# piotrmwojcik/GI-GS

Measured on AMD Instinct MI355X. Metric: train-step renders/sec (fwd+bwd, G-buffer+indirect) at 800x800; PSNR vs the CPU oracle, higher is better.
Workload: dtype f32; 1 GPU; C2 (configs[1] TensoIR lego stand-in): 300k surface Gaussians, 800x800, SH deg 2, GI step=16 start=8 delta=0.0625; P=300000, N=640000, M=9, hip_graphs=on, fused_glue=on, gi_march=proj, rasterizer=whole step = 2 hand-captured hipGraphs (fwd, bwd), asynchronous binning

## Files before the change

gi-gs_amd/csrc/api.hip:

```cpp
#include <cstdarg>
#include <cstdio>
#include <cstdlib>
#include <cstring>
#include <map>
#include <algorithm>
#include <new>
#include <mutex>
#include <vector>

#include "../../include/gigs_hip.h"
#include "gigs_common.h"

namespace {

thread_local char g_err[512] = "";

int fail(int code, const char* fmt, ...) {
  va_list ap;
  va_start(ap, fmt);
  vsnprintf(g_err, sizeof(g_err), fmt, ap);
  va_end(ap);
  return code;
}

// ... 67 lines not shown
  const char* b = getenv("GIGS_BINNING");
  o.binning_legacy = (b && strcmp(b, "legacy") == 0) ? 1 : 0;
  o.bucket_max_mean = env_int("GIGS_BUCKET_MAX_MEAN", gigs::kBucketMaxMeanList);
  const char* ll = getenv("GIGS_LONG_LISTS");
  o.long_lists = (ll && ll[0]) ? (ll[0] == '1' ? 1 : 0) : -1;
  o.bucket_target = std::max(256, env_int("GIGS_BUCKET_TARGET", 1536));
  o.bin_bands = std::max(0, env_int("GIGS_BIN_BANDS", 0));
  o.blend_cull = env_int("GIGS_BLEND_CULL", 1) != 0;
  o.pre_bwd_sh_skip = env_int("GIGS_PRE_BWD_SH_SKIP", 1) != 0;
  o.gi_march = 4;
  if (const char* e = getenv("GIGS_GI_MARCH")) {
    if (strcmp(e, "exact") == 0) o.gi_march = 0;
  }
  o.gi_cert = env_int("GIGS_GI_CERT", 1) != 0;
  o.gi_interleave = env_int("GIGS_GI_INTERLEAVE", 1) != 0;
  o.gi_tile_log2w = env_int("GIGS_GI_TILE_LOG2W", 3);
  if (o.gi_tile_log2w < 0 || o.gi_tile_log2w > 6) o.gi_tile_log2w = 3;
  o.gi_zero_rays = env_int("GIGS_GI_ZERO_RAYS", 0) != 0;
  o.spec_max8 = env_int("GIGS_SPEC_MAX8", 128);
  o.spec_max16 = env_int("GIGS_SPEC_MAX16", 1500);
  o.shade_lds_floats = env_int("GIGS_SHADE_LDS_FLOATS", 30 * 1024);
  o.shade_bwd_blocks = std::max(0, env_int("GIGS_SHADE_BWD_BLOCKS", 0));
  o.shade_bwd_rows = env_int("GIGS_SHADE_BWD_ROWS", 0) != 0;
  return o;
}
const gigs::Ctx& ctx_of(const gigs_ctx* c) { return c ? *reinterpret_cast<const gigs::Ctx*>(c) : gigs::default_ctx(); }

struct ProfRec { int stage; hipEvent_t a, b; };
std::mutex g_prof_mu;
bool g_prof_on = false;
std::vector<ProfRec> g_prof_recs;
std::vector<hipEvent_t> g_prof_pool;

hipEvent_t prof_event() {
  if (!g_prof_pool.empty()) {
    hipEvent_t e = g_prof_pool.back();
    g_prof_pool.pop_back();
    return e;
  }
  hipEvent_t e;
  hipEventCreate(&e);
  return e;
}

struct StageScope {
  hipStream_t s;
// ... 81 lines not shown
  char* p = base;
  gigs::ImageState s = gigs::ImageState::fromChunk(p, N, T);
  const void* ptrs[] = {s.final_T, s.n_contrib, s.ranges, s.tile_order};
  if (which < 0 || which >= 4) return -1;
  return (long long)((const char*)ptrs[which] - base);
}

gigs_ctx* gigs_ctx_create(void) {
  gigs::Ctx* c = new (std::nothrow) gigs::Ctx(gigs::default_ctx());
  if (!c) fail(GIGS_ERR_ALLOC, "gigs_ctx_create: out of host memory");
  return reinterpret_cast<gigs_ctx*>(c);
}
void gigs_ctx_destroy(gigs_ctx* ctx) { delete reinterpret_cast<gigs::Ctx*>(ctx); }

int gigs_ctx_get_options(const gigs_ctx* ctx, gigs_options* out) {
  if (!out || out->struct_bytes < (int)sizeof(gigs_options)) return fail(GIGS_ERR_INVALID, "gigs_ctx_get_options: set struct_bytes = sizeof(gigs_options)");
  const gigs::Options& o = ctx_of(ctx).opt;
  out->struct_bytes = (int)sizeof(gigs_options);
  out->binning_legacy = o.binning_legacy; out->bucket_max_mean = o.bucket_max_mean; out->long_lists = o.long_lists;
  out->bucket_target = o.bucket_target; out->bin_bands = o.bin_bands; out->blend_cull = o.blend_cull; out->pre_bwd_sh_skip = o.pre_bwd_sh_skip;
  out->gi_march = o.gi_march; out->gi_cert = o.gi_cert; out->gi_interleave = o.gi_interleave;
  out->gi_tile_log2w = o.gi_tile_log2w; out->gi_zero_rays = o.gi_zero_rays; out->spec_max8 = o.spec_max8;
  out->spec_max16 = o.spec_max16; out->shade_lds_floats = o.shade_lds_floats; out->shade_bwd_blocks = o.shade_bwd_blocks;
  out->shade_bwd_rows = o.shade_bwd_rows;
  return 0;
}
int gigs_ctx_set_options(gigs_ctx* ctx, const gigs_options* in) {
  if (!ctx) return fail(GIGS_ERR_INVALID, "gigs_ctx_set_options: the default context is immutable, create one");
  if (!in || in->struct_bytes < (int)sizeof(gigs_options)) return fail(GIGS_ERR_INVALID, "gigs_ctx_set_options: set struct_bytes = sizeof(gigs_options)");
  if (in->gi_march != 0 && in->gi_march != 4) return fail(GIGS_ERR_INVALID, "gi_march must be 0 (exact) or 4 (proj)");
  if (in->gi_tile_log2w < 0 || in->gi_tile_log2w > 6) return fail(GIGS_ERR_INVALID, "gi_tile_log2w must be 0..6");
  if (in->long_lists < -1 || in->long_lists > 1) return fail(GIGS_ERR_INVALID, "long_lists must be -1, 0 or 1");
  if (in->bucket_target < 256 || in->bucket_max_mean < 0 || in->bin_bands < 0 || in->bin_bands > 64)
    return fail(GIGS_ERR_INVALID, "bucket_target >= 256, bucket_max_mean >= 0, 0 <= bin_bands <= 64");
  if (in->spec_max8 < 0 || in->spec_max16 < in->spec_max8) return fail(GIGS_ERR_INVALID, "0 <= spec_max8 <= spec_max16");
  if (in->shade_lds_floats < 0 || in->shade_bwd_blocks < 0) return fail(GIGS_ERR_INVALID, "shade_lds_floats, shade_bwd_blocks >= 0");
  gigs::Options& o = reinterpret_cast<gigs::Ctx*>(ctx)->opt;
  o.binning_legacy = in->binning_legacy != 0; o.bucket_max_mean = in->bucket_max_mean; o.long_lists = in->long_lists;
  o.bucket_target = in->bucket_target; o.bin_bands = in->bin_bands; o.blend_cull = in->blend_cull != 0; o.pre_bwd_sh_skip = in->pre_bwd_sh_skip != 0;
  o.gi_march = in->gi_march; o.gi_cert = in->gi_cert != 0; o.gi_interleave = in->gi_interleave != 0;
  o.gi_tile_log2w = in->gi_tile_log2w; o.gi_zero_rays = in->gi_zero_rays != 0; o.spec_max8 = in->spec_max8;
  o.spec_max16 = in->spec_max16; o.shade_lds_floats = in->shade_lds_floats; o.shade_bwd_blocks = in->shade_bwd_blocks;
  o.shade_bwd_rows = in->shade_bwd_rows != 0;
  return 0;
}
int gigs_ctx_set_reuse_binning(gigs_ctx* ctx, int on) {
  if (!ctx) return fail(GIGS_ERR_INVALID, "gigs_ctx_set_reuse_binning: the default context is immutable, create one");
  reinterpret_cast<gigs::Ctx*>(ctx)->reuse_binning = on != 0;
  return 0;
}
int gigs_ctx_set_split_sh(gigs_ctx* ctx, const float* sh_rest) {
  if (!ctx) return fail(GIGS_ERR_INVALID, "gigs_ctx_set_split_sh: the default context is immutable, create one");
  reinterpret_cast<gigs::Ctx*>(ctx)->sh_rest = sh_rest;
  return 0;
}
int gigs_ctx_set_materials_only(gigs_ctx* ctx, void* violations) {
  if (!ctx) return fail(GIGS_ERR_INVALID, "gigs_ctx_set_materials_only: the default context is immutable, create one");
  reinterpret_cast<gigs::Ctx*>(ctx)->materials_only = reinterpret_cast<unsigned*>(violations);
  return 0;
}
int gigs_ctx_set_blend_begin_event(gigs_ctx* ctx, void* hip_event) {
  if (!ctx) return fail(GIGS_ERR_INVALID, "gigs_ctx_set_blend_begin_event: the default context is immutable, create one");
  reinterpret_cast<gigs::Ctx*>(ctx)->blend_begin_event = hip_event;
  return 0;
}

// ... 499 lines not shown
```

gi-gs_amd/csrc/gigs_common.h:

```cpp
#pragma once
#include <hip/hip_runtime.h>
#include <stdint.h>

#define GIGS_BLOCK_X 16
#define GIGS_BLOCK_Y 16
#define GIGS_TILE (GIGS_BLOCK_X * GIGS_BLOCK_Y)
#define GIGS_BREC_F4 5
#define GIGS_GREC 20

namespace gigs {

struct v3 { float x, y, z; };
struct v4 { float x, y, z, w; };

__device__ __forceinline__ v3 operator+(v3 a, v3 b) { return {a.x + b.x, a.y + b.y, a.z + b.z}; }
__device__ __forceinline__ v3 operator-(v3 a, v3 b) { return {a.x - b.x, a.y - b.y, a.z - b.z}; }
__device__ __forceinline__ v3 operator*(v3 a, float s) { return {a.x * s, a.y * s, a.z * s}; }
__device__ __forceinline__ float dot3(v3 a, v3 b) { return a.x * b.x + a.y * b.y + a.z * b.z; }
__device__ __forceinline__ v3 cross3(v3 a, v3 b) {
  return {a.y * b.z - a.z * b.y, a.z * b.x - a.x * b.z, a.x * b.y - a.y * b.x};
}
__device__ __forceinline__ v3 normalize3(v3 v) {
  float inv = 1.0f / sqrtf(dot3(v, v));
  return v * inv;
// ... 162 lines not shown
inline size_t required_bytes(A... a) {
  char* p = nullptr;
  S::fromChunk(p, a...);
  return reinterpret_cast<size_t>(p) + kAlign;
}

struct Options {
  int binning_legacy;
  int bucket_max_mean;
  int long_lists;
  int bucket_target;
  int bin_bands;
  int blend_cull;
  int pre_bwd_sh_skip;
  int gi_march;
  int gi_cert;
  int gi_interleave;
  int gi_tile_log2w;
  int gi_zero_rays;
  int spec_max8, spec_max16;
  int shade_lds_floats;
  int shade_bwd_blocks;
  int shade_bwd_rows;
};
struct Ctx {
  Options opt;
  unsigned async_capacity;
  unsigned* async_counters;
  void* blend_begin_event;
  int reuse_binning;
  unsigned* materials_only;
  const float* sh_rest;
};
const Options& default_options();
const Ctx& default_ctx();

struct FwdArgs {
  int P, D, M, W, H;
  unsigned gx, gy;
  float focal_x, focal_y, tan_fovx, tan_fovy, scale_modifier;
  const float *means3D, *shs, *colors_precomp, *opacities, *normal, *albedo, *roughness,
      *metallic, *scales, *rotations, *cov3D_precomp, *viewmatrix, *projmatrix, *cam_pos,
      *background;
  int argmax_depth, inference;
  const float* shs_rest;
};
// ... 72 lines not shown
```

gi-gs_amd/csrc/pbr.hip:

```cpp
#include <cmath>
#include <cstdlib>
#include <cstring>
#include <map>
#include <mutex>
#include <vector>

#include "gigs_common.h"
#include "pixel_ops.h"

namespace gigs {

__device__ __forceinline__ v3 safe_normalize(v3 v) {
  const float l = sqrtf(v.x * v.x + v.y * v.y + v.z * v.z);
  return l > 0.0f ? v3{v.x / l, v.y / l, v.z / l} : v3{0, 0, 0};
}
__device__ __forceinline__ v3 cube_dir_raw(float fx, float fy, int side) {
  switch (side) {
    case 0: return {1, -fy, -fx};
    case 1: return {-1, -fy, fx};
    case 2: return {fx, 1, fy};
    case 3: return {fx, -1, -fy};
    case 4: return {fx, -fy, 1};
    default: return {-fx, -fy, -1};
  }
// ... 449 lines not shown
static int spec_lanes_for(const Options& o, int avg_window) {
  return (avg_window > 0 && avg_window <= o.spec_max8) ? 8 : (avg_window > 0 && avg_window <= o.spec_max16) ? 16 : 64;
}

template <bool kBackward, bool kNorm>
static void launch_specular_apply(const Options& o, int res, int avg_window, const float* src, const float* bounds,
                                  const uint32_t* offsets, const float* W, float* dst, float* wsum_out, hipStream_t s) {
  const int total = 6 * res * res;
  const int max8 = o.spec_max8, max16 = o.spec_max16;
  if (avg_window > 0 && avg_window <= max8) {
    const int waves = (total + 7) / 8;
    hipLaunchKernelGGL((specular_apply_kernel<kBackward, kNorm, 8>), dim3((waves + 3) / 4), dim3(256), 0, s, res, src,
                       bounds, offsets, W, dst, wsum_out);
  } else if (avg_window > 0 && avg_window <= max16) {
    const int waves = (total + 3) / 4;
    hipLaunchKernelGGL((specular_apply_kernel<kBackward, kNorm, 16>), dim3((waves + 3) / 4), dim3(256), 0, s, res, src,
                       bounds, offsets, W, dst, wsum_out);
  } else {
    hipLaunchKernelGGL((specular_apply_kernel<kBackward, kNorm, 64>), dim3((total + 3) / 4), dim3(256), 0, s, res, src,
                       bounds, offsets, W, dst, wsum_out);
  }
}

__device__ __forceinline__ int cube_face_uv(float x, float y, float z, float& u, float& v) {
  const float ax = fabsf(x), ay = fabsf(y), az = fabsf(z);
  int idx;
  float c;
  if (az > fmaxf(ax, ay)) { idx = 4; c = z; }
  else if (ay > ax) { idx = 2; c = y; y = z; }
  else { idx = 0; c = x; x = z; }
  if (c < 0.f) idx += 1;
  const float m = (1.0f / fabsf(c)) * 0.5f;
  const float m0 = (idx == 0 || idx == 5) ? -m : m;
  const float m1 = (idx != 2) ? -m : m;
  u = x * m0 + 0.5f;
  v = y * m1 + 0.5f;
  if (!isfinite(u) || !isfinite(v)) return -1;
  u = fminf(fmaxf(u, 0.f), 1.f);
  v = fminf(fmaxf(v, 0.f), 1.f);
  return idx;
}

struct Taps { int idx[4]; float w[4]; };

__device__ __forceinline__ bool cube_taps(int res, float dx, float dy, float dz, Taps& t) {
  float u, v;
// ... 802 lines not shown
  if (n_levels <= 0 || n_levels > 8 || !levels) return gigs_internal_fail(GIGS_ERR_INVALID, "specular_cubemap_multi_w: bad level count");
  gigs::SpecLevels L;
  L.n = n_levels;
  int blocks = 0;
  for (int i = 0; i < n_levels; i++) {
    const gigs_spec_level& a = levels[i];
    if (a.res <= 0 || !a.src || !a.bounds || !a.offsets || !a.weights || !a.dst || (!backward && !a.wsum))
      return gigs_internal_fail(GIGS_ERR_INVALID, "specular_cubemap_multi_w: bad level");
    gigs::SpecLevel& v = L.lv[i];
    v.N = a.res; v.lanes = gigs::spec_lanes_for(o, a.avg_window); v.block_begin = blocks;
    v.src = a.src; v.bounds = a.bounds; v.offsets = a.offsets; v.W = a.weights; v.dst = a.dst; v.wsum_out = a.wsum;
    const int total = 6 * a.res * a.res;
    const int waves = v.lanes == 64 ? total : (total + (64 / v.lanes) - 1) / (64 / v.lanes);
    blocks += (waves + 3) / 4;
  }
  void* tok; gigs_internal_stage_begin(backward ? 17 : 16, stream, &tok);
  if (backward) hipLaunchKernelGGL(gigs::specular_apply_multi_kernel<true>, dim3(blocks), dim3(256), 0, (hipStream_t)stream, L);
  else hipLaunchKernelGGL(gigs::specular_apply_multi_kernel<false>, dim3(blocks), dim3(256), 0, (hipStream_t)stream, L);
  gigs_internal_stage_end(tok);
  PBR_CHECK_LAUNCH();
  return 0;
}

int gigs_cubemap_mip_fwd(int res_out, int channels, const float* in, float* out, void* stream) {
  if (res_out <= 0 || channels <= 0 || !in || !out) return gigs_internal_fail(GIGS_ERR_INVALID, "cubemap_mip_fwd: bad argument");
  void* tok; gigs_internal_stage_begin(16, stream, &tok);
  hipLaunchKernelGGL(gigs::cubemap_mip_fwd_kernel, dim3((6 * res_out * res_out * channels + 255) / 256), dim3(256), 0, (hipStream_t)stream, res_out, channels, in, out);
  gigs_internal_stage_end(tok);
  PBR_CHECK_LAUNCH();
  return 0;
}

int gigs_cubemap_mip_bwd(int res_out, const float* dout, float* din, void* stream) {
  if (res_out <= 0 || !dout || !din) return gigs_internal_fail(GIGS_ERR_INVALID, "cubemap_mip_bwd: bad argument");
  const int res = 2 * res_out;
  void* tok; gigs_internal_stage_begin(17, stream, &tok);
  hipLaunchKernelGGL(gigs::cubemap_mip_bwd_kernel, dim3((6 * res * res + 255) / 256), dim3(256), 0, (hipStream_t)stream, res_out, dout, din, (const float*)nullptr,
                     (const float*)nullptr);
  gigs_internal_stage_end(tok);
  PBR_CHECK_LAUNCH();
  return 0;
}

int gigs_cubemap_mip_bwd_add(int res_out, const float* dout, const float* add, float* din, void* stream) {
  if (res_out <= 0 || !dout || !add || !din) return gigs_internal_fail(GIGS_ERR_INVALID, "cubemap_mip_bwd_add: bad argument");
  const int res = 2 * res_out;
// ... 268 lines not shown
```

gi-gs_amd/gigs_lib.py:

```python
from __future__ import annotations

import ctypes as C
import functools
import os
import threading

_HERE = os.path.dirname(os.path.abspath(__file__))
LIB_PATH = os.environ.get("GIGS_LIB", os.path.join(_HERE, "libgigs_hip.so"))

ALLOC_FN = C.CFUNCTYPE(C.c_void_p, C.c_size_t, C.c_void_p)

_f = C.c_void_p
_i = C.c_int
_fl = C.c_float

SIGNATURES = {
    "gigs_last_error": (C.c_char_p, []),
    "gigs_build_arch": (C.c_char_p, []),
    "gigs_required_geom": (C.c_size_t, [_i]),
    "gigs_required_image": (C.c_size_t, [_i, _i]),
    "gigs_required_binning": (C.c_size_t, [_i]),
    "gigs_forward": (_i, [C.c_void_p, ALLOC_FN, C.c_void_p, ALLOC_FN, C.c_void_p, ALLOC_FN, C.c_void_p,
                          _i, _i, _i, _f, _i, _i,
                          _f, _f, _f, _f, _f, _f, _f, _f,
# ... 26 lines not shown
                      C.c_void_p]),
    "gigs_gi_scratch_bytes": (C.c_size_t, [_i, _i]),
    "gigs_ssao_ex": (_i, [C.c_void_p, _i, _i, _fl, _fl, _fl, _fl, _fl, _fl, _i, _i, _f, _f, _f, _f, C.c_void_p]),
    "gigs_ssr_ex": (_i, [C.c_void_p, _i, _i, _fl, _fl, _fl, _fl, _fl, _fl, _i, _i, _f, _f, _f, _f, _f, _f, _f, _f, _f, _f,
                         C.c_void_p]),
    "gigs_ssr_hits": (_i, [C.c_void_p, _i, _i, _fl, _fl, _fl, _fl, _fl, _fl, _i, _i, _f, _f, _f, _f, _f, _f, _f, _f, _f,
                           _i, _f, _f, _f, C.c_uint, _f, C.c_void_p]),
    "gigs_ssr_multi": (_i, [C.c_void_p, _i, _i, _i, _fl, _fl, _fl, _fl, _fl, _fl, _i, _i, _f, _f, _f, _f, _f, _f, _f, _f, _f,
                            _f, C.c_void_p]),
    "gigs_ssr_apply": (_i, [_i, _i, _fl, _f, _f, _f, _f, _f, _f, _f, _f, _f, _f, C.c_void_p]),
    "gigs_median3x3": (_i, [_i, _i, _i, _f, _f, C.c_void_p]),
    "gigs_median3x3_backward": (_i, [_i, _i, _i, _f, _f, _f, C.c_void_p]),
    "gigs_bilateral3x3": (_i, [_i, _i, _i, _fl, _fl, _fl, _f, _f, C.c_void_p]),
    "gigs_diffuse_cubemap_fwd": (_i, [_i, _f, _f, C.c_void_p]),
    "gigs_diffuse_cubemap_bwd": (_i, [_i, _f, _f, C.c_void_p]),
    "gigs_specular_bounds": (_i, [_i, _fl, _f, C.c_void_p]),
    "gigs_specular_cubemap_fwd": (_i, [_i, _f, _f, _fl, _fl, _f, C.c_void_p]),
    "gigs_specular_cubemap_bwd": (_i, [_i, _f, _f, _fl, _fl, _f, C.c_void_p]),
    "gigs_specular_weights": (_i, [_i, _f, _f, _fl, _fl, _i, _f, C.c_void_p]),
    "gigs_specular_weights_divide": (_i, [_i, _f, _f, _f, _f, _f, C.c_void_p]),
    "gigs_specular_cubemap_fwd_w": (_i, [C.c_void_p, _i, _f, _f, _f, _f, _i, _f, _f, C.c_void_p]),
    "gigs_specular_cubemap_bwd_w": (_i, [C.c_void_p, _i, _f, _f, _f, _i, _f, _i, _f, C.c_void_p]),
    "gigs_specular_cubemap_multi_w": (_i, [C.c_void_p, _i, C.c_void_p, _i, C.c_void_p]),
    "gigs_cubemap_mip_fwd": (_i, [_i, _i, _f, _f, C.c_void_p]),
    "gigs_cubemap_mip_bwd_add": (_i, [_i, _f, _f, _f, C.c_void_p]),
    "gigs_cubemap_mip_bwd_add2": (_i, [_i, _f, _f, _f, _f, C.c_void_p]),
    "gigs_cubemap_mip_bwd": (_i, [_i, _f, _f, C.c_void_p]),
    "gigs_shade_fwd": (_i, [_i, _i, _f, _f, _f, _f, _f, _f, _f, _f, _f, _i, _i, C.POINTER(C.c_void_p),
                            C.POINTER(C.c_int), _f, _i, _i, _i, _i, _f, _f, _f, _f, C.c_void_p]),
    "gigs_shade_bwd": (_i, [_i, _i, _f, _f, _f, _f, _f, _f, _f, _f, _i, _i, C.POINTER(C.c_void_p),
                            C.POINTER(C.c_int), _f, _i, _i, _i, _i, _f, _f, _f, _f, _f, _f, _f, _f,
                            C.POINTER(C.c_void_p), C.c_void_p]),
    "gigs_shade_fwd_ex": (_i, [C.c_void_p, _i, _i, _f, _f, _f, _f, _f, _f, _f, _f, _f, _i, _i, C.POINTER(C.c_void_p),
                               C.POINTER(C.c_int), _f, _i, _i, _i, _i, _f, _f, _f, _f, C.c_void_p, C.c_void_p]),
    "gigs_shade_fwd_multi": (_i, [C.c_void_p, _i, _i, _i, _f, _f, _f, _f, _f, _f, _f, C.POINTER(C.c_void_p), _i, _i,
                                  C.POINTER(C.c_void_p), C.POINTER(C.c_int), _f, _i, _i, _i, _i, _f, _f, C.c_void_p]),
    "gigs_shade_bwd_ex": (_i, [C.c_void_p, _i, _i, _f, _f, _f, _f, _f, _f, _f, _f, _i, _i, C.POINTER(C.c_void_p),
                               C.POINTER(C.c_int), _f, _i, _i, _i, _i, _f, _f, _f, _f, _f, _f, _f, _f,
                               C.POINTER(C.c_void_p), C.c_void_p, C.c_void_p]),
    "gigs_gbuffer_post": (_i, [_i, _i, _f, _f, _f, _f, _f, _f, _f, C.c_void_p]),
    "gigs_gbuffer_post_pad": (_i, [_i, _i, _f, _f, _f, _f, _f, _f, _f, _f, _f, _f, _f, _f, C.c_void_p]),
    "gigs_gbuffer_post_bwd": (_i, [_i, _i, _f, _f, _f, _f, _f, C.c_void_p]),
    "gigs_normalize_mask": (_i, [_i, _i, _f, _f, _f, C.c_void_p]),
    "gigs_nonzero_mask": (_i, [_i, _i, _f, _f, C.c_void_p]),
    "gigs_stage2_loss_fwd": (_i, [_i, _i, _f, _f, _f, _f, _f, _f, _f, _f, _f, C.c_void_p]),
    "gigs_stage2_loss_bwd": (_i, [_i, _i, _f, _f, _f, _f, _f, _f, _f, _f, _f, _f, C.c_void_p]),
# ... 44 lines not shown
    "gigs_stream_delay": (_i, [C.c_uint, C.c_void_p]),
    "gigs_ctx_set_async_binning": (_i, [C.c_void_p, _i, C.c_void_p]),
    "gigs_ctx_create": (C.c_void_p, []),
    "gigs_ctx_destroy": (None, [C.c_void_p]),
    "gigs_ctx_get_options": (_i, [C.c_void_p, C.c_void_p]),
    "gigs_ctx_set_options": (_i, [C.c_void_p, C.c_void_p]),
    "gigs_profile_begin": (None, []),
    "gigs_profile_end": (_i, [C.POINTER(C.c_float), C.POINTER(C.c_int), _i]),
    "gigs_profile_stage_name": (C.c_char_p, [_i]),
}

class ShadeExt(C.Structure):
    _fields_ = [("planar", C.c_int), ("rough_scale", C.c_float), ("rough_bias", C.c_float),
                ("out_F0", C.c_void_p), ("out_linear", C.c_void_p), ("out_roughness", C.c_void_p),
                ("g_albedo_mul_a", C.c_void_p), ("g_albedo_mul_b", C.c_void_p),
                ("g_roughness_add", C.c_void_p), ("g_metallic_add", C.c_void_p),
                ("g_scale", C.c_void_p), ("lamb_mask", C.c_void_p), ("lamb_acc4", C.c_void_p)]


class Options(C.Structure):
    _fields_ = [(n, C.c_int) for n in (
        "struct_bytes", "binning_legacy", "bucket_max_mean", "long_lists", "bucket_target", "bin_bands", "blend_cull",
        "pre_bwd_sh_skip", "gi_march", "gi_cert", "gi_interleave", "gi_tile_log2w", "gi_zero_rays", "spec_max8",
        "spec_max16", "shade_lds_floats", "shade_bwd_blocks", "shade_bwd_rows")]


OPTION_NAMES = tuple(n for n, _ in Options._fields_ if n != "struct_bytes")
GI_MARCHES = {0: "exact", 4: "proj"}
_GI_MARCH_VALUES = {name: value for value, name in GI_MARCHES.items()}


class SpecLevel(C.Structure):
    _fields_ = [("res", C.c_int), ("avg_window", C.c_int), ("src", C.c_void_p), ("bounds", C.c_void_p),
                ("offsets", C.c_void_p), ("weights", C.c_void_p), ("dst", C.c_void_p), ("wsum", C.c_void_p)]


class AdamGroup(C.Structure):
    _fields_ = [("param", C.c_void_p), ("grad", C.c_void_p), ("exp_avg", C.c_void_p), ("exp_avg_sq", C.c_void_p),
                ("n", C.c_longlong), ("lr", C.c_double), ("step", C.c_int)]


class ActivationRaw(C.Structure):
    _fields_ = [(n, C.c_void_p) for n in ("f_dc", "f_rest", "opacity", "normal", "albedo", "roughness", "metallic",
                                          "scaling", "rotation")]


class ActivationOut(C.Structure):
    _fields_ = [(n, C.c_void_p) for n in ("shs", "opacities", "normal", "albedo", "roughness", "metallic", "scales",
                                          "rotations")]


class GatherTensor(C.Structure):
    _fields_ = [("src", C.c_void_p), ("dst", C.c_void_p), ("row_floats", C.c_int), ("zero_new", C.c_int)]


class PackDesc(C.Structure):
    _fields_ = [("src", C.c_void_p), ("dst", C.c_void_p), ("lohi", C.c_void_p), ("channels", C.c_int), ("height", C.c_int),
                ("width", C.c_int), ("dst_x", C.c_int), ("dst_stride", C.c_int), ("bias", C.c_float)]


class FilterDesc(C.Structure):
    _fields_ = [("sheet", C.c_void_p), ("out", C.c_void_p), ("height", C.c_int), ("width", C.c_int), ("stride", C.c_int),
                ("reserved", C.c_int)]


MAX_IMAGES = 4096
MINMAX_SCRATCH_FLOATS = 512

_lib = None


class GigsError(RuntimeError):
    pass


def lib():
    global _lib
    if _lib is None:
        if not os.path.exists(LIB_PATH):
            raise ImportError(
                f"{LIB_PATH} not found: build it with `python gi-gs_amd/build.py` "
                "(hipcc, --offload-arch=gfx950). There is no CPU fallback.")
        l = C.CDLL(LIB_PATH)
        for name, (res, args) in SIGNATURES.items():
            fn = getattr(l, name)
            fn.restype = res
            fn.argtypes = args
        _lib = l
# ... 179 lines not shown
```

gi-gs_amd/pbr/renderutils/ops.py:

```python
from __future__ import annotations

import os

import numpy as np
import torch

import gigs_lib

_lib = gigs_lib.lib()


def _stream() -> int:
    return torch.cuda.current_stream().cuda_stream


def _gpu(t: torch.Tensor, name: str) -> torch.Tensor:
    if not t.is_cuda:
        raise RuntimeError(f"{name} must be a CUDA/HIP tensor: pbr.renderutils (gigs-hip) has no CPU path")
    return t.contiguous().float()


class _diffuse_cubemap_func(torch.autograd.Function):
    @staticmethod
    def forward(ctx, cubemap):
# ... 145 lines not shown
        dev = cs[0].device
        outs, wsums, arr = [], [], (gigs_lib.SpecLevel * len(cs))()
        for i, (c, (bounds, tables)) in enumerate(zip(cs, meta)):
            res = c.shape[1]
            out = torch.empty((6, res, res, 3), dtype=torch.float32, device=dev)
            wsum = torch.empty((6, res, res, 1), dtype=torch.float32, device=dev)
            outs.append(out)
            wsums.append(wsum)
            arr[i] = gigs_lib.SpecLevel(res, _avg_window(tables, res), c.data_ptr(), bounds.data_ptr(), tables[0].data_ptr(),
                                        tables[1].data_ptr(), out.data_ptr(), wsum.data_ptr())
        with torch.cuda.device(dev):
            gigs_lib.check(_lib.gigs_specular_cubemap_multi_w(gigs_lib.ctx_ptr(), len(cs), C.cast(arr, C.c_void_p), 0, _stream()),
                           "specular_cubemap_multi_w")
        ctx.meta = meta
        ctx.lib_ctx = gigs_lib.current()
        ctx.shapes = [c.shape[1] for c in cs]
        return tuple(outs)

    @staticmethod
    @gigs_lib.with_forward_context
    def backward(ctx, *douts):
        import ctypes as C
        dev = next(d for d in douts if d is not None).device
        gs, arr, keep = [], (gigs_lib.SpecLevel * len(douts))(), []
        for i, (d, res, (bounds, tables)) in enumerate(zip(douts, ctx.shapes, ctx.meta)):
            d = torch.zeros((6, res, res, 3), dtype=torch.float32, device=dev) if d is None else _gpu(d, "dout")
            keep.append(d)
            g = torch.empty((6, res, res, 3), dtype=torch.float32, device=dev)
            gs.append(g)
            arr[i] = gigs_lib.SpecLevel(res, _avg_window(tables, res), d.data_ptr(), bounds.data_ptr(), tables[0].data_ptr(),
                                        tables[3].data_ptr(), g.data_ptr(), None)
        with torch.cuda.device(dev):
            if bwd_head_start_ns > 0:
                gigs_lib.check(_lib.gigs_stream_delay(int(bwd_head_start_ns), _stream()), "stream_delay")
            gigs_lib.check(_lib.gigs_specular_cubemap_multi_w(gigs_lib.ctx_ptr(), len(douts), C.cast(arr, C.c_void_p), 1, _stream()),
                           "specular_cubemap_multi_w")
        return (None, *gs)


def specular_cubemap_levels(mips, roughnesses, cutoff=0.99):
    if os.environ.get("GIGS_SPEC_MULTI", "1") != "1" or torch.is_anomaly_enabled() or not mips[0].is_cuda:
        return None
    meta = []
    for m, r in zip(mips, roughnesses):
        _, bounds = _ndf_bounds(m.shape[1], r, cutoff, m.device)
        tables = _weight_tables(m.shape[1], r, cutoff, m.device)
        if tables is None or len(tables) < 4 or tables[3] is None:
            return None
        meta.append((bounds, tables))
    return list(_specular_levels.apply(meta, *mips))


_TABLE_MAX_BYTES = float(os.environ.get("GIGS_SPEC_TABLE_MAX_GB", "8")) * 1e9
_weightTables = {}


def _weight_tables(res, roughness, cutoff, device):
    key = (res, roughness, cutoff, str(device))
    if key not in _weightTables:
        cos_cut, bounds = _ndf_bounds(res, roughness, cutoff, device)
        b = bounds.view(-1, 6, 4)
        w = torch.where(b[..., 0] <= b[..., 1], b[..., 1] - b[..., 0] + 1, torch.zeros_like(b[..., 0]))
        h = torch.where(b[..., 2] <= b[..., 3], b[..., 3] - b[..., 2] + 1, torch.zeros_like(b[..., 0]))
        cnt = (w * h).to(torch.int64).reshape(-1)
        total = int(cnt.sum().item())
        used = sum(t[1].numel() * (12 if t[3] is not None else 8) for t in _weightTables.values() if t is not None)
        if total == 0 or total >= 2 ** 31 or used + total * 8 > _TABLE_MAX_BYTES:
            _weightTables[key] = None
        else:
            offsets = (torch.cumsum(cnt, 0) - cnt).to(torch.int32).contiguous()
            tabs = []
            with torch.cuda.device(device):
                for swap in (0, 1):
                    wt = torch.empty(total, dtype=torch.float32, device=device)
                    gigs_lib.check(_lib.gigs_specular_weights(res, bounds.data_ptr(), offsets.data_ptr(), float(roughness),
                                                              float(cos_cut), swap, wt.data_ptr(), _stream()),
                                   "specular_weights")
                    tabs.append(wt)
            scaled = None
            if os.environ.get("GIGS_SPEC_PRESCALED", "1") == "1" and used + total * 12 <= _TABLE_MAX_BYTES:
                with torch.cuda.device(device):
                    ones = torch.ones((6, res, res, 3), dtype=torch.float32, device=device)
                    tmp = torch.empty_like(ones)
                    wsum = torch.empty((6, res, res), dtype=torch.float32, device=device)
                    gigs_lib.check(_lib.gigs_specular_cubemap_fwd_w(gigs_lib.ctx_ptr(), res, ones.data_ptr(), bounds.data_ptr(),
                                                                    offsets.data_ptr(), tabs[0].data_ptr(), 0,
                                                                    tmp.data_ptr(), wsum.data_ptr(), _stream()),
                                   "specular_cubemap_fwd_w")
                    scaled = torch.empty(total, dtype=torch.float32, device=device)
                    gigs_lib.check(_lib.gigs_specular_weights_divide(res, bounds.data_ptr(), offsets.data_ptr(),
                                                                     tabs[1].data_ptr(), wsum.data_ptr(), scaled.data_ptr(),
                                                                     _stream()), "specular_weights_divide")
            _weightTables[key] = (offsets, tabs[0], tabs[1], scaled)
    return _weightTables[key]


def specular_cubemap(cubemap, roughness, cutoff=0.99, use_python=False):
    assert cubemap.shape[0] == 6 and cubemap.shape[1] == cubemap.shape[2], \
        "Bad shape for cubemap tensor: %s" % str(cubemap.shape)
    if use_python:
        assert False
    if not cubemap.is_cuda:
        raise RuntimeError("cubemap must be a CUDA/HIP tensor: pbr.renderutils (gigs-hip) has no CPU path")
    cos_cut, bounds = _ndf_bounds(cubemap.shape[1], roughness, cutoff, cubemap.device)
    tables = _weight_tables(cubemap.shape[1], roughness, cutoff, cubemap.device)
    if tables is not None and not torch.is_anomaly_enabled():
        return _specular_cubemap_normalized.apply(cubemap, bounds, tables)
    out = _specular_cubemap.apply(cubemap, roughness, cos_cut, bounds, tables)
    if torch.is_anomaly_enabled():
        assert not torch.isnan(out).any(), "Output of specular_cubemap contains inf or NaN"
    return out[..., 0:3] / out[..., 3:]
```

include/gigs_hip.h:

```cpp
#ifndef GIGS_HIP_H_
#define GIGS_HIP_H_

#include <stddef.h>
#include <stdint.h>

#ifdef __cplusplus
extern "C" {
#endif

#define GIGS_OK 0
#define GIGS_ERR_INVALID (-1)
#define GIGS_ERR_HIP (-2)
#define GIGS_ERR_ALLOC (-3)

typedef char* (*gigs_alloc_fn)(size_t nbytes, void* user);

const char* gigs_last_error(void);
const char* gigs_build_arch(void);

typedef struct gigs_ctx gigs_ctx;
typedef struct gigs_options {
  int struct_bytes;
  int binning_legacy;
  int bucket_max_mean;
  int long_lists;
  int bucket_target;
  int bin_bands;
  int blend_cull;
  int pre_bwd_sh_skip;
  int gi_march;
  int gi_cert;
  int gi_interleave;
  int gi_tile_log2w;
  int gi_zero_rays;
  int spec_max8;
  int spec_max16;
  int shade_lds_floats;
  int shade_bwd_blocks;
  int shade_bwd_rows;
} gigs_options;
gigs_ctx* gigs_ctx_create(void);
void gigs_ctx_destroy(gigs_ctx* ctx);
int gigs_ctx_get_options(const gigs_ctx* ctx, gigs_options* out);
int gigs_ctx_set_options(gigs_ctx* ctx, const gigs_options* in);

size_t gigs_required_geom(int P);
size_t gigs_required_image(int width, int height);
size_t gigs_required_binning(int num_rendered);

int gigs_forward(gigs_ctx* ctx, gigs_alloc_fn geometryBuffer, void* geom_user, gigs_alloc_fn binningBuffer,
                 void* binning_user, gigs_alloc_fn imageBuffer, void* image_user, int P, int D, int M,
                 const float* background, int width, int height, const float* means3D,
                 const float* shs, const float* colors_precomp, const float* opacities,
                 const float* normal, const float* albedo, const float* roughness,
                 const float* metallic, const float* scales, float scale_modifier,
                 const float* rotations, const float* cov3D_precomp, const float* viewmatrix,
                 const float* projmatrix, const float* cam_pos, float tan_fovx, float tan_fovy,
                 int prefiltered, int argmax_depth, int inference, float* out_color,
                 float* out_opacity, float* out_depth, float* out_normal, float* out_normal_view,
                 float* out_pos, float* out_albedo, float* out_roughness, float* out_metallic,
                 int* radii, int debug, void* stream);

// ... 71 lines not shown
                              float costheta_cutoff, float* out, void* stream);
int gigs_specular_cubemap_bwd(int res, const float* bounds, const float* grad_out, float roughness,
                              float costheta_cutoff, float* grad_cubemap, void* stream);
int gigs_specular_weights(int res, const float* bounds, const uint32_t* offsets, float roughness,
                          float costheta_cutoff, int swap_roles, float* weights, void* stream);
int gigs_specular_weights_divide(int res, const float* bounds, const uint32_t* offsets, const float* weights,
                                 const float* texel_divisor, float* out_weights, void* stream);
int gigs_specular_cubemap_fwd_w(gigs_ctx* ctx, int res, const float* cubemap, const float* bounds, const uint32_t* offsets,
                                const float* weights, int avg_window, float* out, float* wsum_out, void* stream);
int gigs_specular_cubemap_bwd_w(gigs_ctx* ctx, int res, const float* bounds, const uint32_t* offsets,
                                const float* weights_swapped, int avg_window, const float* grad_out,
                                int grad_is_rgb, float* grad_cubemap, void* stream);

typedef struct gigs_spec_level {
  int res, avg_window;
  const float* src;
  const float* bounds;
  const uint32_t* offsets;
  const float* weights;
  float* dst;
  float* wsum;
} gigs_spec_level;
int gigs_specular_cubemap_multi_w(gigs_ctx* ctx, int n_levels, const gigs_spec_level* levels, int backward, void* stream);
int gigs_cubemap_mip_fwd(int res_out, int channels, const float* in, float* out, void* stream);
int gigs_cubemap_mip_bwd(int res_out, const float* dout, float* din, void* stream);
int gigs_cubemap_mip_bwd_add(int res_out, const float* dout, const float* add, float* din, void* stream);
int gigs_cubemap_mip_bwd_add2(int res_out, const float* dout, const float* dout2, const float* add, float* din, void* stream);

int gigs_shade_fwd(int H, int W, const float* normals, const float* view_dirs, const float* albedo,
                   const float* roughness, const uint8_t* mask, const float* occlusion,
                   const float* metallic, const float* background, const float* diffuse, int diffuse_res,
                   int n_levels, const float* const* spec, const int* spec_res, const float* lut,
                   int lut_w, int lut_h, int tone, int gamma, float* render_rgb, float* diffuse_rgb,
                   float* specular_rgb, float* diffuse_light, void* stream);
int gigs_shade_bwd(int H, int W, const float* normals, const float* view_dirs, const float* albedo,
                   const float* roughness, const uint8_t* mask, const float* occlusion,
                   const float* metallic, const float* diffuse, int diffuse_res, int n_levels,
                   const float* const* spec, const int* spec_res, const float* lut, int lut_w, int lut_h,
                   int tone, int gamma, const float* g_render, const float* g_diffuse_rgb,
                   const float* g_specular_rgb, const float* g_diffuse_light, float* d_albedo,
                   float* d_roughness, float* d_metallic, float* d_diffuse, float* const* d_spec,
                   void* stream);

typedef struct gigs_shade_ext {
  int planar;
  float rough_scale, rough_bias;
// ... 195 lines not shown
```

Measured before the change: 346.1 renders/s.

## Add sparse scatter path for specular cubemap backward with dense fallback

Adds a census kernel that zeroes the gradient output and compacts the list of nonzero output texels of the specular prefilter gradient. A scatter kernel then pushes only those texels' gradients through the forward weight tables, using an LDS-tiled accumulation for wide filters. The dense gather backward still runs as a fallback when the nonzero count exceeds a capacity set as a fraction of texels. This avoids the dense per-texel gather when incoming gradients are sparse, at the cost of atomics, extra launches and device state buffers that must work under graph capture.

After: 352.7 renders/s (median of 6 runs). 1.02x the previous value.

```diff
diff --git a/gi-gs_amd/csrc/api.hip b/gi-gs_amd/csrc/api.hip
--- a/gi-gs_amd/csrc/api.hip
+++ b/gi-gs_amd/csrc/api.hip
@@ -113,6 +113,9 @@
   o.shade_lds_floats = env_int("GIGS_SHADE_LDS_FLOATS", 30 * 1024);
   o.shade_bwd_blocks = std::max(0, env_int("GIGS_SHADE_BWD_BLOCKS", 0));
   o.shade_bwd_rows = env_int("GIGS_SHADE_BWD_ROWS", 0) != 0;
+  o.spec_sparse = env_int("GIGS_SPEC_SPARSE", 1) != 0;
+  o.spec_sparse_permille = env_int("GIGS_SPEC_SPARSE_PERMILLE", 37);
+  if (o.spec_sparse_permille < 0 || o.spec_sparse_permille > 1000) o.spec_sparse_permille = 37;
   return o;
 }
 const gigs::Ctx& ctx_of(const gigs_ctx* c) { return c ? *reinterpret_cast<const gigs::Ctx*>(c) : gigs::default_ctx(); }
@@ -240,7 +243,7 @@
   out->gi_march = o.gi_march; out->gi_cert = o.gi_cert; out->gi_interleave = o.gi_interleave;
   out->gi_tile_log2w = o.gi_tile_log2w; out->gi_zero_rays = o.gi_zero_rays; out->spec_max8 = o.spec_max8;
   out->spec_max16 = o.spec_max16; out->shade_lds_floats = o.shade_lds_floats; out->shade_bwd_blocks = o.shade_bwd_blocks;
-  out->shade_bwd_rows = o.shade_bwd_rows;
+  out->shade_bwd_rows = o.shade_bwd_rows; out->spec_sparse = o.spec_sparse; out->spec_sparse_permille = o.spec_sparse_permille;
   return 0;
 }
 int gigs_ctx_set_options(gigs_ctx* ctx, const gigs_options* in) {
@@ -253,13 +256,14 @@
     return fail(GIGS_ERR_INVALID, "bucket_target >= 256, bucket_max_mean >= 0, 0 <= bin_bands <= 64");
   if (in->spec_max8 < 0 || in->spec_max16 < in->spec_max8) return fail(GIGS_ERR_INVALID, "0 <= spec_max8 <= spec_max16");
   if (in->shade_lds_floats < 0 || in->shade_bwd_blocks < 0) return fail(GIGS_ERR_INVALID, "shade_lds_floats, shade_bwd_blocks >= 0");
+  if (in->spec_sparse_permille < 0 || in->spec_sparse_permille > 1000) return fail(GIGS_ERR_INVALID, "0 <= spec_sparse_permille <= 1000");
   gigs::Options& o = reinterpret_cast<gigs::Ctx*>(ctx)->opt;
   o.binning_legacy = in->binning_legacy != 0; o.bucket_max_mean = in->bucket_max_mean; o.long_lists = in->long_lists;
   o.bucket_target = in->bucket_target; o.bin_bands = in->bin_bands; o.blend_cull = in->blend_cull != 0; o.pre_bwd_sh_skip = in->pre_bwd_sh_skip != 0;
   o.gi_march = in->gi_march; o.gi_cert = in->gi_cert != 0; o.gi_interleave = in->gi_interleave != 0;
   o.gi_tile_log2w = in->gi_tile_log2w; o.gi_zero_rays = in->gi_zero_rays != 0; o.spec_max8 = in->spec_max8;
   o.spec_max16 = in->spec_max16; o.shade_lds_floats = in->shade_lds_floats; o.shade_bwd_blocks = in->shade_bwd_blocks;
-  o.shade_bwd_rows = in->shade_bwd_rows != 0;
+  o.shade_bwd_rows = in->shade_bwd_rows != 0; o.spec_sparse = in->spec_sparse != 0; o.spec_sparse_permille = in->spec_sparse_permille;
   return 0;
 }
 int gigs_ctx_set_reuse_binning(gigs_ctx* ctx, int on) {
diff --git a/gi-gs_amd/csrc/gigs_common.h b/gi-gs_amd/csrc/gigs_common.h
--- a/gi-gs_amd/csrc/gigs_common.h
+++ b/gi-gs_amd/csrc/gigs_common.h
@@ -208,6 +208,8 @@
   int shade_lds_floats;
   int shade_bwd_blocks;
   int shade_bwd_rows;
+  int spec_sparse;
+  int spec_sparse_permille;
 };
 struct Ctx {
   Options opt;
diff --git a/gi-gs_amd/csrc/pbr.hip b/gi-gs_amd/csrc/pbr.hip
--- a/gi-gs_amd/csrc/pbr.hip
+++ b/gi-gs_amd/csrc/pbr.hip
@@ -495,6 +495,239 @@
   }
 }
 
+struct SparseLevel {
+  int total, cap, block_begin, group_begin, N;
+  int vec;
+  int chunks;
+  int lds;
+  const float* src;
+  float* dst;
+  const float* bounds;
+  const uint32_t* offsets;
+  const float* Wfwd;
+  const float* wsum;
+  int* list;
+};
+struct SparseLevels { int n; SparseLevel lv[8]; };
+
+constexpr int kCensusPerThread = 4;
+
+__global__ void __launch_bounds__(256) specular_census_kernel(SparseLevels L, int* __restrict__ state) {
+  int k = 0;
+#pragma unroll
+  for (int i = 1; i < 8; i++)
+    if (i < L.n && (int)blockIdx.x >= L.lv[i].block_begin) k = i;
+  const SparseLevel& v = L.lv[k];
+  const int lane = threadIdx.x & 63;
+  const int t0 = (((int)blockIdx.x - v.block_begin) * 256 + (int)threadIdx.x) * kCensusPerThread;
+  bool nz[kCensusPerThread];
+  if (v.vec && t0 + kCensusPerThread <= v.total) {
+    const float4* s4 = reinterpret_cast<const float4*>(v.src + 3 * (size_t)t0);
+    float4* d4 = reinterpret_cast<float4*>(v.dst + 3 * (size_t)t0);
+    const float4 a = s4[0], b = s4[1], c = s4[2];
+    nz[0] = a.x != 0.0f || a.y != 0.0f || a.z != 0.0f;
+    nz[1] = a.w != 0.0f || b.x != 0.0f || b.y != 0.0f;
+    nz[2] = b.z != 0.0f || b.w != 0.0f || c.x != 0.0f;
+    nz[3] = c.y != 0.0f || c.z != 0.0f || c.w != 0.0f;
+    const float4 z = {0.0f, 0.0f, 0.0f, 0.0f};
+    d4[0] = z; d4[1] = z; d4[2] = z;
+  } else {
+#pragma unroll
+    for (int j = 0; j < kCensusPerThread; j++) {
+      nz[j] = false;
+      if (t0 + j < v.total) {
+        const float* s = v.src + 3 * (size_t)(t0 + j);
+        float* d = v.dst + 3 * (size_t)(t0 + j);
+        nz[j] = s[0] != 0.0f || s[1] != 0.0f || s[2] != 0.0f;
+        d[0] = 0.0f; d[1] = 0.0f; d[2] = 0.0f;
+      }
+    }
+  }
+  unsigned long long m[kCensusPerThread];
+  int wave_total = 0;
+#pragma unroll
+  for (int j = 0; j < kCensusPerThread; j++) { m[j] = __ballot(nz[j]); wave_total += __popcll(m[j]); }
+  __shared__ int wave_base[5];
+  const int wave = threadIdx.x >> 6;
+  if (lane == 0) wave_base[wave] = wave_total;
+  __syncthreads();
+  if (threadIdx.x == 0) {
+    const int t01 = wave_base[0] + wave_base[1], t012 = t01 + wave_base[2], all = t012 + wave_base[3];
+    const int first = all ? atomicAdd(state + k, all) : 0;
+    wave_base[3] = first + t012; wave_base[2] = first + t01; wave_base[1] = first + wave_base[0]; wave_base[0] = first;
+  }
+  __syncthreads();
+  if (wave_total == 0) return;
+  int base = wave_base[wave];
+  const unsigned long long below = (1ull << lane) - 1ull;
+#pragma unroll
+  for (int j = 0; j < kCensusPerThread; j++) {
+    const int slot = base + __popcll(m[j] & below);
+    if (nz[j] && slot < v.cap) v.list[slot] = t0 + j;
+    base += __popcll(m[j]);
+  }
+}
+
+constexpr int kScatterU = 2;
+constexpr int kLdsTile = 32;
+constexpr int kLdsParts = 8;
+constexpr int kLdsWide = 16;
+
+__global__ void __launch_bounds__(256) specular_scatter_kernel(SparseLevels L, int* __restrict__ state) {
+  const int lane = threadIdx.x & 63;
+  const int group = (int)blockIdx.x * 4 + ((int)threadIdx.x >> 6);
+  if (blockIdx.x == 0 && threadIdx.x < 8 && (int)threadIdx.x < L.n) {
+    const int c = state[threadIdx.x];
+    state[8 + threadIdx.x] = c <= L.lv[threadIdx.x].cap ? 1 : 0;
+    state[16 + threadIdx.x] = c;
+  }
+  int k = 0;
+#pragma unroll
+  for (int i = 1; i < 8; i++)
+    if (i < L.n && group >= L.lv[i].group_begin) k = i;
+  const SparseLevel& v = L.lv[k];
+  const int count = state[k];
+  if (count > v.cap) return;
+  if (v.lds) {
+    __shared__ float img[kLdsTile * kLdsTile * 3];
+    const int N = v.N, nt = (N + kLdsTile - 1) / kLdsTile, bl = (group - v.group_begin) >> 2;
+    const int face = bl % 6, tile = (bl / 6) % (nt * nt), part = bl / (6 * nt * nt);
+    const int tx0 = (tile % nt) * kLdsTile, ty0 = (tile / nt) * kLdsTile;
+    const int tx1 = min(tx0 + kLdsTile, N) - 1, ty1 = min(ty0 + kLdsTile, N) - 1;
+    const int wave = (int)threadIdx.x >> 6;
+    for (int i = threadIdx.x; i < kLdsTile * kLdsTile * 3; i += 256) img[i] = 0.0f;
+    __syncthreads();
+    const int listed = min(count, v.cap);
+    for (int slot = part + kLdsParts * wave; slot < listed; slot += kLdsParts * 4) {
+      const int o = __builtin_amdgcn_readfirstlane(v.list[slot]);
+      const float4* b4 = reinterpret_cast<const float4*>(v.bounds + 24 * (size_t)o);
+      int before = 0, xmin = 0, xmax = -1, ymin = 0, ymax = -1;
+#pragma unroll
+      for (int s = 0; s < 6; ++s) {
+        const float4 b = b4[s];
+        const int x0 = (int)b.x, x1 = (int)b.y, y0 = (int)b.z, y1 = (int)b.w;
+        const int cnt = (x0 > x1 || y0 > y1) ? 0 : (x1 - x0 + 1) * (y1 - y0 + 1);
+        if (s < face) before += cnt;
+        if (s == face && cnt) { xmin = x0; xmax = x1; ymin = y0; ymax = y1; }
+      }
+      const int ix0 = max(xmin, tx0), ix1 = min(xmax, tx1), iy0 = max(ymin, ty0), iy1 = min(ymax, ty1);
+      if (ix0 > ix1 || iy0 > iy1) continue;
+      const int wd = xmax - xmin + 1, iw = ix1 - ix0 + 1, ni = iw * (iy1 - iy0 + 1);
+      const float* W = v.Wfwd + v.offsets[6 * (size_t)o] + before;
+      const float ws = v.wsum[o], inv = 1.0f / (float)iw;
+      const float* g = v.src + 3 * (size_t)o;
+      const float g0 = g[0], g1 = g[1], g2 = g[2];
+      for (int i = lane; i < ni; i += 64) {
+        const int ry = (int)(((float)i + 0.5f) * inv), y = iy0 + ry, x = ix0 + (i - ry * iw);
+        const float w = W[(y - ymin) * wd + (x - xmin)];
+        if (!(w >= 0.0f)) continue;
+        float* t = img + 3 * ((y - ty0) * kLdsTile + (x - tx0));
+        const float q = w / ws;
+        const float v0 = q * g0, v1 = q * g1, v2 = q * g2;
+        if (v0 != 0.0f) atomicAdd(t, v0);
+        if (v1 != 0.0f) atomicAdd(t + 1, v1);
+        if (v2 != 0.0f) atomicAdd(t + 2, v2);
+      }
+    }
+    __syncthreads();
+    const int row3 = 3 * (tx1 - tx0 + 1), cells = row3 * (ty1 - ty0 + 1);
+    for (int i = threadIdx.x; i < cells; i += 256) {
+      const int yy = i / row3, xc = i - yy * row3;
+      const float val = img[3 * yy * kLdsTile + xc];
+      if (val != 0.0f) atomicAdd(v.dst + 3 * ((size_t)(face * N + ty0 + yy) * N + tx0) + xc, val);
+    }
+    return;
+  }
+  const int slot = (group - v.group_begin) / v.chunks, chunk = (group - v.group_begin) % v.chunks;
+  if (slot >= count || slot >= v.cap) return;
+  const int o = __builtin_amdgcn_readfirstlane(v.list[slot]);
+  const int N = v.N;
+  int pre[7], wd[6], base[6];
+  float inv[6];
+  pre[0] = 0;
+  const float4* b4 = reinterpret_cast<const float4*>(v.bounds + 24 * (size_t)o);
+#pragma unroll
+  for (int s = 0; s < 6; ++s) {
+    const float4 b = b4[s];
+    const int xmin = (int)b.x, xmax = (int)b.y, ymin = (int)b.z, ymax = (int)b.w;
+    const bool empty = xmin > xmax || ymin > ymax;
+    wd[s] = empty ? 1 : xmax - xmin + 1;
+    inv[s] = 1.0f / (float)wd[s];
+    pre[s + 1] = pre[s] + (empty ? 0 : wd[s] * (ymax - ymin + 1));
+    base[s] = empty ? 0 : (s * N + ymin) * N + xmin;
+  }
+  const int n = pre[6];
+  const float* W = v.Wfwd + v.offsets[6 * (size_t)o];
+  const float ws = v.wsum[o];
+  const float* g = v.src + 3 * (size_t)o;
+  const float g0 = g[0], g1 = g[1], g2 = g[2];
+  const int step = 64 * v.chunks;
+  int from[3];
+  float gch[3];
+#pragma unroll
+  for (int j = 0; j < 3; j++) {
+    const int D = 64 * j + lane, ch = D % 3;
+    from[j] = D / 3;
+    gch[j] = ch == 0 ? g0 : ch == 1 ? g1 : g2;
+  }
+  const int ch0 = lane % 3;
+  for (int c0 = 64 * chunk; c0 < n; c0 += step * kScatterU) {
+    float w[kScatterU];
+#pragma unroll
+    for (int u = 0; u < kScatterU; u++) {
+      const int c = c0 + u * step + lane;
+      w[u] = c < n ? W[c] : -1.0f;
+    }
+#pragma unroll
+    for (int u = 0; u < kScatterU; u++) {
+      if (c0 + u * step >= n) break;
+      const int c = c0 + u * step + lane;
+      float q = -1.0f;
+      int texel = 0;
+      if (w[u] >= 0.0f) {
+        int f = 0;
+#pragma unroll
+        for (int j = 1; j < 6; j++) f += c >= pre[j] ? 1 : 0;
+        int f_pre = pre[0], f_wd = wd[0], f_base = base[0];
+        float f_inv = inv[0];
+#pragma unroll
+        for (int j = 1; j < 6; j++)
+          if (f == j) { f_pre = pre[j]; f_wd = wd[j]; f_base = base[j]; f_inv = inv[j]; }
+        const int loc = c - f_pre;
+        const int row = (int)(((float)loc + 0.5f) * f_inv);
+        texel = f_base + row * N + (loc - row * f_wd);
+        q = w[u] / ws;
+      }
+#pragma unroll
+      for (int j = 0; j < 3; j++) {
+        const float qq = __shfl(q, from[j]);
+        const int tt = __shfl(texel, from[j]);
+        const int ch = ch0 + j >= 3 ? ch0 + j - 3 : ch0 + j;
+        const float val = qq * gch[j];
+        if (!(qq < 0.0f) && val != 0.0f) atomicAdd(v.dst + 3 * (size_t)tt + ch, val);
+      }
+    }
+  }
+}
+
+__global__ void __launch_bounds__(256) specular_apply_multi_bwd_sparse_kernel(SpecLevels L, int* __restrict__ state) {
+  int k = 0;
+#pragma unroll
+  for (int i = 1; i < 8; i++)
+    if (i < L.n && (int)blockIdx.x >= L.lv[i].block_begin) k = i;
+  if (blockIdx.x == 0 && threadIdx.x < 8) state[threadIdx.x] = 0;
+  if (state[8 + k] != 0) return;
+  const SpecLevel& v = L.lv[k];
+  const int block = (int)blockIdx.x - v.block_begin;
+  if (v.lanes == 8) specular_apply_body<true, true, 8>(block, v.N, v.src, v.bounds, v.offsets, v.W, v.dst, v.wsum_out);
+  else if (v.lanes == 16) specular_apply_body<true, true, 16>(block, v.N, v.src, v.bounds, v.offsets, v.W, v.dst, v.wsum_out);
+  else specular_apply_body<true, true, 64>(block, v.N, v.src, v.bounds, v.offsets, v.W, v.dst, v.wsum_out);
+}
+
+static int spec_sparse_capacity(const Options& o, int res) {
+  return (int)((long long)6 * res * res * o.spec_sparse_permille / 1000);
+}
+
 __device__ __forceinline__ int cube_face_uv(float x, float y, float z, float& u, float& v) {
   const float ax = fabsf(x), ay = fabsf(y), az = fabsf(z);
   int idx;
@@ -1343,6 +1576,56 @@
   return 0;
 }
 
+int gigs_spec_sparse_capacity(const gigs_ctx* ctx, int res) {
+  if (res <= 0 || res > 4096) return gigs_internal_fail(GIGS_ERR_INVALID, "spec_sparse_capacity: bad resolution");
+  return gigs::spec_sparse_capacity(*gigs_internal_options(ctx), res);
+}
+
+int gigs_specular_cubemap_multi_bwd_sparse(gigs_ctx* ctx, int n_levels, const gigs_spec_level* levels,
+                                           const float* const* weights_fwd, const float* const* wsum, int* state,
+                                           int* lists, void* stream) {
+  const gigs::Options& o = *gigs_internal_options(ctx);
+  if (!o.spec_sparse) return gigs_specular_cubemap_multi_w(ctx, n_levels, levels, 1, stream);
+  if (n_levels <= 0 || n_levels > 8 || !levels || !weights_fwd || !wsum || !state || !lists)
+    return gigs_internal_fail(GIGS_ERR_INVALID, "specular_cubemap_multi_bwd_sparse: bad argument");
+  gigs::SpecLevels L;
+  gigs::SparseLevels S;
+  L.n = S.n = n_levels;
+  int blocks = 0, census_blocks = 0, groups = 0;
+  size_t list_begin = 0;
+  for (int i = 0; i < n_levels; i++) {
+    const gigs_spec_level& a = levels[i];
+    if (a.res <= 0 || a.res > 4096 || !a.src || !a.bounds || !a.offsets || !a.weights || !a.dst || !weights_fwd[i] || !wsum[i])
+      return gigs_internal_fail(GIGS_ERR_INVALID, "specular_cubemap_multi_bwd_sparse: bad level");
+    gigs::SpecLevel& v = L.lv[i];
+    v.N = a.res; v.lanes = gigs::spec_lanes_for(o, a.avg_window); v.block_begin = blocks;
+    v.src = a.src; v.bounds = a.bounds; v.offsets = a.offsets; v.W = a.weights; v.dst = a.dst; v.wsum_out = a.wsum;
+    const int total = 6 * a.res * a.res;
+    const int waves = v.lanes == 64 ? total : (total + (64 / v.lanes) - 1) / (64 / v.lanes);
+    blocks += (waves + 3) / 4;
+    gigs::SparseLevel& q = S.lv[i];
+    q.total = total; q.cap = gigs::spec_sparse_capacity(o, a.res); q.block_begin = census_blocks; q.group_begin = groups; q.N = a.res;
+    q.vec = ((((uintptr_t)a.src) | ((uintptr_t)a.dst)) & 15) == 0;
+    q.src = a.src; q.dst = a.dst; q.bounds = a.bounds; q.offsets = a.offsets; q.Wfwd = weights_fwd[i]; q.wsum = wsum[i];
+    q.list = lists + list_begin;
+    const int per_block = 256 * gigs::kCensusPerThread;
+    census_blocks += (total + per_block - 1) / per_block;
+    q.chunks = std::min(32, std::max(1, (std::max(1, a.avg_window) + 64 * 2 * gigs::kScatterU - 1) / (64 * 2 * gigs::kScatterU)));
+    q.lds = (long long)a.avg_window * gigs::kLdsWide >= total;
+    const int nt = (a.res + gigs::kLdsTile - 1) / gigs::kLdsTile;
+    groups += q.lds ? 4 * 6 * nt * nt * gigs::kLdsParts : (q.cap * q.chunks + 3) / 4 * 4;
+    list_begin += (size_t)q.cap;
+  }
+  hipStream_t s = (hipStream_t)stream;
+  void* tok; gigs_internal_stage_begin(17, stream, &tok);
+  hipLaunchKernelGGL(gigs::specular_census_kernel, dim3(census_blocks), dim3(256), 0, s, S, state);
+  hipLaunchKernelGGL(gigs::specular_scatter_kernel, dim3(std::max(1, (groups + 3) / 4)), dim3(256), 0, s, S, state);
+  hipLaunchKernelGGL(gigs::specular_apply_multi_bwd_sparse_kernel, dim3(blocks), dim3(256), 0, s, L, state);
+  gigs_internal_stage_end(tok);
+  PBR_CHECK_LAUNCH();
+  return 0;
+}
+
 int gigs_cubemap_mip_fwd(int res_out, int channels, const float* in, float* out, void* stream) {
   if (res_out <= 0 || channels <= 0 || !in || !out) return gigs_internal_fail(GIGS_ERR_INVALID, "cubemap_mip_fwd: bad argument");
   void* tok; gigs_internal_stage_begin(16, stream, &tok);
diff --git a/gi-gs_amd/gigs_lib.py b/gi-gs_amd/gigs_lib.py
--- a/gi-gs_amd/gigs_lib.py
+++ b/gi-gs_amd/gigs_lib.py
@@ -72,6 +72,9 @@
     "gigs_specular_cubemap_fwd_w": (_i, [C.c_void_p, _i, _f, _f, _f, _f, _i, _f, _f, C.c_void_p]),
     "gigs_specular_cubemap_bwd_w": (_i, [C.c_void_p, _i, _f, _f, _f, _i, _f, _i, _f, C.c_void_p]),
     "gigs_specular_cubemap_multi_w": (_i, [C.c_void_p, _i, C.c_void_p, _i, C.c_void_p]),
+    "gigs_spec_sparse_capacity": (_i, [C.c_void_p, _i]),
+    "gigs_specular_cubemap_multi_bwd_sparse": (_i, [C.c_void_p, _i, C.c_void_p, C.POINTER(C.c_void_p), C.POINTER(C.c_void_p),
+                                                    C.c_void_p, C.c_void_p, C.c_void_p]),
     "gigs_cubemap_mip_fwd": (_i, [_i, _i, _f, _f, C.c_void_p]),
     "gigs_cubemap_mip_bwd_add": (_i, [_i, _f, _f, _f, C.c_void_p]),
     "gigs_cubemap_mip_bwd_add2": (_i, [_i, _f, _f, _f, _f, C.c_void_p]),
@@ -162,7 +165,7 @@
     _fields_ = [(n, C.c_int) for n in (
         "struct_bytes", "binning_legacy", "bucket_max_mean", "long_lists", "bucket_target", "bin_bands", "blend_cull",
         "pre_bwd_sh_skip", "gi_march", "gi_cert", "gi_interleave", "gi_tile_log2w", "gi_zero_rays", "spec_max8",
-        "spec_max16", "shade_lds_floats", "shade_bwd_blocks", "shade_bwd_rows")]
+        "spec_max16", "shade_lds_floats", "shade_bwd_blocks", "shade_bwd_rows", "spec_sparse", "spec_sparse_permille")]
 
 
 OPTION_NAMES = tuple(n for n, _ in Options._fields_ if n != "struct_bytes")
@@ -204,6 +207,7 @@
                 ("reserved", C.c_int)]
 
 
+SPEC_SPARSE_STATE_INTS = 32
 MAX_IMAGES = 4096
 MINMAX_SCRATCH_FLOATS = 512
 
diff --git a/gi-gs_amd/pbr/renderutils/ops.py b/gi-gs_amd/pbr/renderutils/ops.py
--- a/gi-gs_amd/pbr/renderutils/ops.py
+++ b/gi-gs_amd/pbr/renderutils/ops.py
@@ -191,7 +191,9 @@
     def backward(ctx, *douts):
         import ctypes as C
         dev = next(d for d in douts if d is not None).device
-        gs, arr, keep = [], (gigs_lib.SpecLevel * len(douts))(), []
+        n = len(douts)
+        gs, arr, keep = [], (gigs_lib.SpecLevel * n)(), []
+        w_fwd, w_sum = (C.c_void_p * n)(), (C.c_void_p * n)()
         for i, (d, res, (bounds, tables)) in enumerate(zip(douts, ctx.shapes, ctx.meta)):
             d = torch.zeros((6, res, res, 3), dtype=torch.float32, device=dev) if d is None else _gpu(d, "dout")
             keep.append(d)
@@ -199,12 +201,59 @@
             gs.append(g)
             arr[i] = gigs_lib.SpecLevel(res, _avg_window(tables, res), d.data_ptr(), bounds.data_ptr(), tables[0].data_ptr(),
                                         tables[3].data_ptr(), g.data_ptr(), None)
+            w_fwd[i], w_sum[i] = tables[1].data_ptr(), tables[4].data_ptr()
         with torch.cuda.device(dev):
             if bwd_head_start_ns > 0:
                 gigs_lib.check(_lib.gigs_stream_delay(int(bwd_head_start_ns), _stream()), "stream_delay")
-            gigs_lib.check(_lib.gigs_specular_cubemap_multi_w(gigs_lib.ctx_ptr(), len(douts), C.cast(arr, C.c_void_p), 1, _stream()),
-                           "specular_cubemap_multi_w")
+            state, lists = _sparse_buffers(tuple(ctx.shapes), dev)
+            gigs_lib.check(_lib.gigs_specular_cubemap_multi_bwd_sparse(gigs_lib.ctx_ptr(), n, C.cast(arr, C.c_void_p), w_fwd, w_sum,
+                                                                       None if state is None else state.data_ptr(),
+                                                                       None if lists is None else lists.data_ptr(), _stream()),
+                           "specular_cubemap_multi_bwd_sparse")
         return (None, *gs)
+
+
+_sparseBuffers = {}
+_sparseSpares = {}
+_sparseCaptured = []
+
+
+def _new_sparse_pair(caps, device):
+    return (torch.zeros(gigs_lib.SPEC_SPARSE_STATE_INTS, dtype=torch.int32, device=device),
+            torch.empty(max(1, sum(caps)), dtype=torch.int32, device=device))
+
+
+def _sparse_buffers(shapes, device):
+    if not gigs_lib.current().option("spec_sparse"):
+        return None, None
+    caps = tuple(gigs_lib.check(_lib.gigs_spec_sparse_capacity(gigs_lib.ctx_ptr(), r), "spec_sparse_capacity") for r in shapes)
+    chain = (shapes, caps, str(device))
+    if torch.cuda.is_current_stream_capturing():
+        spares = _sparseSpares.get(chain)
+        pair = spares.pop() if spares else _new_sparse_pair(caps, device)
+        _sparseCaptured.append(pair)
+    else:
+        key = chain + (_stream(),)
+        if key not in _sparseBuffers:
+            _sparseBuffers[key] = _new_sparse_pair(caps, device)
+        if not _sparseSpares.get(chain):
+            _sparseSpares[chain] = [_new_sparse_pair(caps, device)]
+        pair = _sparseBuffers[key]
+    _sparseLast[(shapes, str(device))] = pair[0]
+    return pair
+
+
+_sparseLast = {}
+
+
+def spec_sparse_report(shapes, device=None):
+    device = torch.device("cuda", torch.cuda.current_device()) if device is None else device
+    state = _sparseLast.get((tuple(shapes), str(device)))
+    if state is None:
+        return None
+    torch.cuda.synchronize(device)
+    v = state.cpu().tolist()
+    return [(bool(v[8 + i]), v[16 + i]) for i in range(len(shapes))]
 
 
 def specular_cubemap_levels(mips, roughnesses, cutoff=0.99):
@@ -246,7 +295,7 @@
                                                               float(cos_cut), swap, wt.data_ptr(), _stream()),
                                    "specular_weights")
                     tabs.append(wt)
-            scaled = None
+            scaled = wsum = None
             if os.environ.get("GIGS_SPEC_PRESCALED", "1") == "1" and used + total * 12 <= _TABLE_MAX_BYTES:
                 with torch.cuda.device(device):
                     ones = torch.ones((6, res, res, 3), dtype=torch.float32, device=device)
@@ -260,7 +309,7 @@
                     gigs_lib.check(_lib.gigs_specular_weights_divide(res, bounds.data_ptr(), offsets.data_ptr(),
                                                                      tabs[1].data_ptr(), wsum.data_ptr(), scaled.data_ptr(),
                                                                      _stream()), "specular_weights_divide")
-            _weightTables[key] = (offsets, tabs[0], tabs[1], scaled)
+            _weightTables[key] = (offsets, tabs[0], tabs[1], scaled, wsum if scaled is not None else None)
     return _weightTables[key]
 
 
diff --git a/include/gigs_hip.h b/include/gigs_hip.h
--- a/include/gigs_hip.h
+++ b/include/gigs_hip.h
@@ -38,6 +38,8 @@
   int shade_lds_floats;
   int shade_bwd_blocks;
   int shade_bwd_rows;
+  int spec_sparse;
+  int spec_sparse_permille;
 } gigs_options;
 gigs_ctx* gigs_ctx_create(void);
 void gigs_ctx_destroy(gigs_ctx* ctx);
@@ -155,6 +157,11 @@
   float* wsum;
 } gigs_spec_level;
 int gigs_specular_cubemap_multi_w(gigs_ctx* ctx, int n_levels, const gigs_spec_level* levels, int backward, void* stream);
+#define GIGS_SPEC_SPARSE_STATE_INTS 32
+int gigs_spec_sparse_capacity(const gigs_ctx* ctx, int res);
+int gigs_specular_cubemap_multi_bwd_sparse(gigs_ctx* ctx, int n_levels, const gigs_spec_level* levels,
+                                           const float* const* weights_fwd, const float* const* wsum, int* state,
+                                           int* lists, void* stream);
 int gigs_cubemap_mip_fwd(int res_out, int channels, const float* in, float* out, void* stream);
 int gigs_cubemap_mip_bwd(int res_out, const float* dout, float* din, void* stream);
 int gigs_cubemap_mip_bwd_add(int res_out, const float* dout, const float* add, float* din, void* stream);
```
